# Healthcare-Robotics/assistive-gym

Measured on AMD Instinct MI355X. Metric: env_steps_per_sec, higher is better.
Workload: dtype f32; 1 GPU; FeedingJaco-v1, 4096 lockstep envs per MI355X, random-policy rollout, 5 simulation steps per env step, 50 PGS sweeps; envs_per_gpu=4096, global_envs=4096, reset_pool=256, reset=pool, parallelism=env-sharded x1, obs_allgather=False

## Files before the change

### __graft_entry__.py

```python
import os
import subprocess
import sys

ROOT = os.path.dirname(os.path.abspath(__file__))
if ROOT not in sys.path:
    sys.path.insert(0, ROOT)


def build():
    from assistive_gym_amd.build import build as build_lib
    build_lib(force=True)
    build_lib(out=os.path.join(ROOT, 'assistive_gym_amd', 'lib', 'variants', 'lvs.so'), extra=('-DAGX_PGS_LV=3',), only=['FEEDING'])
    build_lib(out=os.path.join(ROOT, 'assistive_gym_amd', 'lib', 'variants', 'scan4.so'), extra=('-DAGX_GJK_SCAN_WIDE=0', '-DAGX_GJK_SCAN_ONE=0'), only=['FEEDING'])
    subprocess.check_call(['make', '-C', os.path.join(ROOT, 'oracle')], stdout=subprocess.DEVNULL)
    if os.path.isdir('/root/reference/assistive_gym/envs/assets'):
        from assistive_gym_amd.model import compiler
        compiler.main()
    import assistive_gym_amd
    from assistive_gym_amd import libagx
    L = libagx.load()
    missing = [e for e in libagx.EXPORTS if not hasattr(L, e)]
    assert not missing, missing


def smoke():
    import numpy as np
    sys.path.insert(0, os.path.join(ROOT, 'tests'))
    from assistive_gym_amd import libagx
    from assistive_gym_amd.blob import ModelBlob
    from assistive_gym_amd.vec_env import build_reset_pool
    from oracle_lib import Oracle
    libagx.check(libagx.load().agx_selftest(0), 'agx_selftest')
    n = 64
    for model in ('feeding_jaco', 'bed_bathing_sawyer'):
        blob = ModelBlob.load(model)
        states = build_reset_pool(blob, n, seed=1001)
        st = libagx.Stepper(blob, n)
        st.set_state(states)
        actions = np.random.RandomState(0).uniform(-1, 1, (n, blob.act_dim)).astype(np.float32)
        obs, rew, done, info = st.step_host(actions)
        o = Oracle(blob)
        worst = 0.0
        for i in range(8):
            o_obs, o_rew, _, o_info = o.step(states[i].copy(), actions[i])
            worst = max(worst, float(np.abs(obs[i] - o_obs).max()), abs(float(rew[i]) - o_rew))
        assert np.isfinite(obs).all() and np.isfinite(rew).all()
# ... 10 lines not shown
```

### assistive_gym_amd/csrc/agx_collide.h

```cpp
#pragma once

namespace agx {

struct Cand { v3 pa, pb, n; float dist, gap; };
constexpr float GJK_FAR_MARGIN = 1e-4f;

AGX_DEV void make_shape(const Ctx& c, int col, v3 shift, gjk_shape& s) {
  s.n = CLI(c, col, AGX_C_NVERT);
  s.v = c.bf + c.o_vert + 3 * CLI(c, col, AGX_C_VOFF);
  v3 p; body_xf(c, CLI(c, col, AGX_C_BODY), s.R, p);
  s.p = p - shift; s.box = false;
  s.c = mul(s.R, mk3(CLF(c, col, AGX_C_AABB_C), CLF(c, col, AGX_C_AABB_C + 1), CLF(c, col, AGX_C_AABB_C + 2))) + s.p;
}
AGX_DEV bool narrowphase(const Ctx& c, int ca, int cb, float limit, Cand& out, bool has) {
  const float* AB = c.lds + L_ARENA;
  gjk_shape sa, sb;
  sa.v = nullptr; sa.n = 0; sa.box = false; sa.c = mk3(0.f, 0.f, 0.f); sb.v = nullptr; sb.n = 0; sb.box = false; sb.c = sa.c;
  v3 shift = mk3(0.f, 0.f, 0.f);
  float ra = 0.f, rb = 0.f;
  bool ok = has;
  if (has) {
    shift = mk3(0.5f * (AB[ABS * ca] + AB[ABS * ca + 3]), 0.5f * (AB[ABS * ca + 1] + AB[ABS * ca + 4]), 0.5f * (AB[ABS * ca + 2] + AB[ABS * ca + 5]));
    make_shape(c, ca, shift, sa); make_shape(c, cb, shift, sb);
    if (CLI(c, cb, AGX_C_BODY) == AGX_BODY_WORLD && sb.n == 8 && (CLI(c, cb, AGX_C_TAG) == AGX_TAG_TABLE || CLI(c, cb, AGX_C_TAG) == AGX_TAG_PLANE)) {
// ... 259 lines not shown
  const int na_live = nlive[0], nb = nlive[1];
  wave_sync();
  const int npairs = na_live * nb * rep;
  for (int base = 0; base < npairs; base += 64) {
    const int p = base + lane; bool ok = p < npairs;
    const int pq = ok ? p / rep : 0, sub = ok ? p - pq * rep : 0;
    const int ai = pq / nb; const int a = LIST[ai], b = LIST[128 + pq - ai * nb];
    ok = ok && (!same || b > a) && (sub == 0 || (face_box(c, b) && CLI(c, a, AGX_C_NVERT) >= 2));
    if (ok && no_adjacent) {
      const int la = CLI(c, a, AGX_C_BODY), lb = CLI(c, b, AGX_C_BODY);
      if (la == lb) ok = false;
      else if (la >= 0 && la < AGX_BODY_ROBOT_BASE && lb >= 0 && lb < AGX_BODY_ROBOT_BASE && (RBI(c, la, AGX_R_PARENT) == lb || RBI(c, lb, AGX_R_PARENT) == la)) ok = false;
    }
    if (ok) for (int q = 0; q < 3; q++) if (AB[ABS * a + q] > AB[ABS * b + 3 + q] + mg || AB[ABS * b + q] > AB[ABS * a + 3 + q] + mg) ok = false;
    if (ok) { const float reach = mg + rel_travel(c, a, b) + 1e-5f; ok = !sphere_box_apart(c, a, b, reach) && (CLI(c, a, AGX_C_NVERT) == 1 || !sphere_box_apart(c, b, a, reach)); }
    const uint64_t m = wave_ballot(ok);
    const int slot = wn + wave_rank(m);
    if (ok && slot < WL_CAP) WL[slot] = a | (b << 9) | (g << 18) | (sub << 24);
    wn += popc64(m);
  }
  wave_sync();
  return wn;
}

AGX_DEV void collide(Ctx& c) {
  float* L = c.lds; float* AB = L + L_ARENA; const int lane = c.lane;
  const float brk = PRM(c, AGX_P_CONTACT_BREAK), slack = PRM(c, AGX_P_CONTACT_SLACK);
  CollideState cs; cs.ncon = 0; cs.near_mask = 0; cs.overflow = 0; cs.nqpt = 0;
  cs.maxc = (int)PRM(c, AGX_P_MAX_CONTACTS); if (cs.maxc > MAX_CON) cs.maxc = MAX_CON;
  long long ct0 = c.timing ? wave_clock() : 0, ct1;
#define AGX_CTICK(k) if (c.timing) { ct1 = wave_clock(); c.tm[k] += ct1 - ct0; ct0 = ct1; }
  if (lane < MAX_DOF + MAX_FREE) {
    v3 w = mk3(0, 0, 0), v = w;
    if (lane < MAX_DOF) { if (lane < c.ndof) for (int d = lane; d >= 0; d = RBI(c, d, AGX_R_PARENT)) { const float qd = L[L_VEL + d]; w = w + qd * ld3(L + L_S + 6 * d); v = v + qd * ld3(L + L_S + 6 * d + 3); } }
    else if (lane - MAX_DOF < c.nfree) {
      const int fb = lane - MAX_DOF, o = c.ndof + 6 * fb;
      w = ld3(L + L_VEL + o + 3);
      v = ld3(L + L_VEL + o) + cross(w, ld3(L + L_MISC + M_REF) - ld3(L + L_ST + c.s_free + 13 * fb));
    }
    L[L_WMAG + lane] = sqrtf(dot(w, w));
    st3(AB + A_TW + 6 * lane, w); st3(AB + A_TW + 6 * lane + 3, v);
  }
  wave_sync();
  for (int col = lane; col < c.ncoll; col += 64) {
    const int code = CLI(c, col, AGX_C_BODY);
    m3 R; v3 p; body_xf(c, code, R, p);
    v3 cl = mk3(CLF(c, col, AGX_C_AABB_C), CLF(c, col, AGX_C_AABB_C + 1), CLF(c, col, AGX_C_AABB_C + 2));
    v3 hl = mk3(CLF(c, col, AGX_C_AABB_H), CLF(c, col, AGX_C_AABB_H + 1), CLF(c, col, AGX_C_AABB_H + 2));
    v3 cw = mul(R, cl) + p; float r = CLF(c, col, AGX_C_RADIUS);
    v3 vc = point_velocity(c, code, cw);
    const float wmag = body_wmag(c, code);
    const float grow = (sqrtf(dot(vc, vc)) + wmag * (sqrtf(dot(hl, hl)) + r)) * c.dt;
    for (int k = 0; k < 3; k++) {
      float h = fabsf(R.a[3 * k]) * hl.x + fabsf(R.a[3 * k + 1]) * hl.y + fabsf(R.a[3 * k + 2]) * hl.z + r;
      AB[ABS * col + k] = comp(cw, k) - h - grow; AB[ABS * col + 3 + k] = comp(cw, k) + h + grow;
    }
    AB[ABS * col + 6] = grow;
  }
  wave_sync();
  AGX_CTICK(8)
  const int gender = c.ldsi[L_ST + c.s_env + AGX_E_GENDER];
  uint64_t live_groups = 0;
  GroupRegs G; G.a0 = 0; G.a1 = 0; G.b0 = 0; G.b1 = 0; G.flags = 0; G.keep = 0;
  for (int k = 0; k < 3; k++) { G.alo[k] = 0.f; G.ahi[k] = 0.f; G.blo[k] = 0.f; G.bhi[k] = 0.f; }
  {
    const int g = lane; bool live = false;
    if (g < c.ngroup) {
// ... 56 lines not shown
```

### assistive_gym_amd/csrc/agx_ctx.h

```cpp
#pragma once

namespace agx {

#ifndef AGX_MAX_DOF
#define AGX_MAX_DOF 16
#endif
#ifndef AGX_MAX_FREE
#define AGX_MAX_FREE 10
#endif
#ifndef AGX_MAX_BLOCK
#define AGX_MAX_BLOCK 10
#endif
#ifndef AGX_TASK
#define AGX_TASK 0
#endif
#define AGX_HAS_SAMPLER 1
constexpr int MAX_DOF = AGX_MAX_DOF;
constexpr int MAX_FREE = AGX_MAX_FREE;
constexpr int MAX_BLOCK = AGX_MAX_BLOCK;
constexpr int TASK = AGX_TASK;
constexpr int MAX_HUMAN = 20;
constexpr int MAX_CON = 64;
constexpr int MAX_ROWS = 160;
#ifndef AGX_ST_WORDS
// ... 95 lines not shown
  float* lds; int* ldsi;
  int lane;
  int ndof, nfree, nhuman, ncoll, ngroup, nfood, nv;
  int nrobot, nhdof, gender, frozen, s_tremor;
  float limit_scale;
  bool coop;
  int o_params, o_robot, o_free, o_coll, o_vert, o_group, o_task, o_dirs;
  int s_q, s_qd, s_qt, s_free, s_base, s_human, s_env;
  float dt;
  bool hooks;
  int ncon, nrows, first_normal, near_mask, overflow;
  float* gqpt; int nqpt;
  float* dbg;
  float* E; float* H;
  int nent;
  float* gcon;
  long long tm[16]; bool timing;
};

#define PRM(c, k) ((c).bf[(c).o_params + (k)])
#define RREC(c, d) ((d) < (c).nrobot ? (d) : (d) + (c).gender * (c).nhdof)
#define RBF(c, d, k) ((c).bf[(c).o_robot + RREC(c, d) * AGX_R_STRIDE + (k)])
#define RBI(c, d, k) ((c).bi[(c).o_robot + RREC(c, d) * AGX_R_STRIDE + (k)])
#define DLO(c, d) (RBF(c, d, AGX_R_LOWER) * ((RBI(c, d, AGX_R_KIND) & 3) == 1 ? (c).limit_scale : 1.f))
#define DHI(c, d) (RBF(c, d, AGX_R_UPPER) * ((RBI(c, d, AGX_R_KIND) & 3) == 1 ? (c).limit_scale : 1.f))
#define FROZEN(c, d) ((d) < 32 && (((c).frozen >> (d)) & 1))
#define FBF(c, b, k) ((c).bf[(c).o_free + (b) * AGX_F_STRIDE + (k)])
#define CLF(c, i, k) ((c).bf[(c).o_coll + (i) * AGX_C_STRIDE + (k)])
#define CLI(c, i, k) ((c).bi[(c).o_coll + (i) * AGX_C_STRIDE + (k)])
#define GRI(c, g, k) ((c).bi[(c).o_group + (g) * AGX_G_STRIDE + (k)])
#define TKF(c, k) ((c).bf[(c).o_task + (k)])
#define TKI(c, k) ((c).bi[(c).o_task + (k)])

AGX_DEV void ctx_init(Ctx& c, const uint32_t* blob, float* lds, int lane) {
  c.bf = (const float*)blob; c.bi = (const int*)blob; c.lds = lds; c.ldsi = (int*)lds; c.lane = lane;
  const int* h = c.bi;
  c.ndof = h[AGX_H_NDOF]; c.nfree = h[AGX_H_NFREE]; c.nhuman = h[AGX_H_NHUMAN]; c.ncoll = h[AGX_H_NCOLL];
  c.ngroup = h[AGX_H_NGROUP]; c.nfood = h[AGX_H_NFOOD]; c.nv = c.ndof + 6 * c.nfree;
  c.o_params = h[AGX_H_OFF_PARAMS]; c.o_robot = h[AGX_H_OFF_ROBOT]; c.o_free = h[AGX_H_OFF_FREE]; c.o_coll = h[AGX_H_OFF_COLL];
  c.o_vert = h[AGX_H_OFF_VERT]; c.o_group = h[AGX_H_OFF_GROUP]; c.o_task = h[AGX_H_OFF_TASK]; c.o_dirs = h[AGX_H_OFF_DIRS];
  c.s_q = h[AGX_H_S_Q]; c.s_qd = h[AGX_H_S_QD]; c.s_qt = h[AGX_H_S_QT]; c.s_free = h[AGX_H_S_FREE]; c.s_base = h[AGX_H_S_BASE];
  c.s_human = h[AGX_H_S_HUMAN]; c.s_env = h[AGX_H_S_ENV]; c.s_tremor = h[AGX_H_S_TREMOR];
  c.nrobot = h[AGX_H_NROBOT]; c.nhdof = h[AGX_H_NHDOF]; c.gender = 0; c.frozen = 0; c.limit_scale = 1.f; c.coop = false;
  c.dt = PRM(c, AGX_P_DT) / (float)(h[AGX_H_SIM_SUBSTEPS] > 1 ? h[AGX_H_SIM_SUBSTEPS] : 1); c.hooks = true;
  c.ncon = 0; c.nrows = 0; c.first_normal = 0; c.near_mask = 0; c.overflow = 0; c.nent = 0; c.dbg = nullptr; c.E = nullptr; c.H = nullptr; c.gcon = nullptr; c.gqpt = nullptr; c.nqpt = 0;
  c.timing = false; for (int k = 0; k < 16; k++) c.tm[k] = 0;
}

AGX_DEV float dot6p(const float* a, const float* b) { return a[0] * b[0] + a[1] * b[1] + a[2] * b[2] + a[3] * b[3] + a[4] * b[4] + a[5] * b[5]; }
AGX_DEV void body_xf(const Ctx& c, int code, m3& R, v3& p) {
  const float* L = c.lds;
  if (code == AGX_BODY_WORLD) { R.a[0] = 1; R.a[1] = 0; R.a[2] = 0; R.a[3] = 0; R.a[4] = 1; R.a[5] = 0; R.a[6] = 0; R.a[7] = 0; R.a[8] = 1; p = mk3(0, 0, 0); }
  else if (code >= AGX_BODY_HUMAN0) { const float* h = L + L_HUMAN + 12 * (code - AGX_BODY_HUMAN0); p = ld3(h); R = ldm3(h + 3); }
  else if (code >= AGX_BODY_FREE0) { int b = code - AGX_BODY_FREE0; p = ld3(L + L_ST + c.s_free + 13 * b); R = ldm3(L + L_FREER + 9 * b); }
  else if (code == AGX_BODY_ROBOT_BASE) { p = ld3(L + L_BASE); R = ldm3(L + L_BASE + 3); }
  else { p = ld3(L + L_LINKP + 3 * code); R = ldm3(L + L_LINKR + 9 * code); }
}

}
```

### assistive_gym_amd/csrc/agx_dyn.h

```cpp
#pragma once

namespace agx {

AGX_DEV void kinematics(Ctx& c) {
  float* L = c.lds; const int lane = c.lane, n = c.ndof;
  for (int d = 0; d < n; d++) {
    int par = RBI(c, d, AGX_R_PARENT);
    v3 pp; m3 PR;
    if (par == AGX_PARENT_HUMAN_BASE) { pp = ld3(L + L_HUMAN); PR = ldm3(L + L_HUMAN + 3); }
    else if (par < 0) { pp = ld3(L + L_BASE); PR = ldm3(L + L_BASE + 3); } else { pp = ld3(L + L_LINKP + 3 * par); PR = ldm3(L + L_LINKR + 9 * par); }
    v3 tp = mk3(RBF(c, d, AGX_R_TPOS), RBF(c, d, AGX_R_TPOS + 1), RBF(c, d, AGX_R_TPOS + 2));
    m3 Rt = quat_to_m3(RBF(c, d, AGX_R_TQUAT), RBF(c, d, AGX_R_TQUAT + 1), RBF(c, d, AGX_R_TQUAT + 2), RBF(c, d, AGX_R_TQUAT + 3));
    v3 ax = mk3(RBF(c, d, AGX_R_AXIS), RBF(c, d, AGX_R_AXIS + 1), RBF(c, d, AGX_R_AXIS + 2));
    const bool prismatic = RBI(c, d, AGX_R_JTYPE) == 1;
    const float qj = L[L_ST + c.s_q + d];
    m3 R = mul(PR, Rt);
    v3 p = mul(PR, tp) + pp;
    if (prismatic) p = p + qj * mul(R, ax); else R = mul(R, axis_angle_m3(ax, qj));
    wave_sync();
    if (lane == 0) { st3(L + L_LINKP + 3 * d, p); stm3(L + L_LINKR + 9 * d, R); }
    wave_sync();
  }
  {
    int ee = TKI(c, AGX_T_EE_LINK);
    v3 lp = ld3(L + L_LINKP + 3 * ee); m3 LR = ldm3(L + L_LINKR + 9 * ee);
    v3 ep = mul(LR, mk3(TKF(c, AGX_T_EE_POS), TKF(c, AGX_T_EE_POS + 1), TKF(c, AGX_T_EE_POS + 2))) + lp;
    m3 ER = mul(LR, quat_to_m3(TKF(c, AGX_T_EE_QUAT), TKF(c, AGX_T_EE_QUAT + 1), TKF(c, AGX_T_EE_QUAT + 2), TKF(c, AGX_T_EE_QUAT + 3)));
    if (lane == 0) { st3(L + L_MISC + M_REF, lp); st3(L + L_MISC + M_EEP, ep); stm3(L + L_MISC + M_EER, ER); }
  }
  wave_sync();
  const v3 ref = ld3(L + L_MISC + M_REF);
  float* A = L + L_ARENA;
  if (lane < n) {
    const int d = lane;
    v3 p = ld3(L + L_LINKP + 3 * d) - ref; m3 R = ldm3(L + L_LINKR + 9 * d);
    v3 aw = mul(R, mk3(RBF(c, d, AGX_R_AXIS), RBF(c, d, AGX_R_AXIS + 1), RBF(c, d, AGX_R_AXIS + 2)));
    if (RBI(c, d, AGX_R_JTYPE) == 1) { st3(L + L_S + 6 * d, mk3(0.f, 0.f, 0.f)); st3(L + L_S + 6 * d + 3, aw); }
    else { st3(L + L_S + 6 * d, aw); st3(L + L_S + 6 * d + 3, cross(p, aw)); }
    v3 cw = mul(R, mk3(RBF(c, d, AGX_R_COM), RBF(c, d, AGX_R_COM + 1), RBF(c, d, AGX_R_COM + 2))) + p;
    st3(A + A_COMW + 3 * d, cw);
    m3 Il;
    Il.a[0] = RBF(c, d, AGX_R_INERTIA); Il.a[4] = RBF(c, d, AGX_R_INERTIA + 1); Il.a[8] = RBF(c, d, AGX_R_INERTIA + 2);
    Il.a[1] = Il.a[3] = RBF(c, d, AGX_R_INERTIA + 3); Il.a[2] = Il.a[6] = RBF(c, d, AGX_R_INERTIA + 4); Il.a[5] = Il.a[7] = RBF(c, d, AGX_R_INERTIA + 5);
    stm3(A + A_IW + 9 * d, mul_bt(mul(R, Il), R));
  }
  wave_sync();
  if (lane < n) {
    const int d = lane;
    float v[6] = {0, 0, 0, 0, 0, 0};
    for (int k = d; k >= 0; k = RBI(c, k, AGX_R_PARENT)) { float qd = L[L_ST + c.s_qd + k]; for (int j = 0; j < 6; j++) v[j] += L[L_S + 6 * k + j] * qd; }
    float qd = L[L_ST + c.s_qd + d];
    v3 w = mk3(v[0], v[1], v[2]), vo = mk3(v[3], v[4], v[5]);
    v3 sw = qd * ld3(L + L_S + 6 * d), sv = qd * ld3(L + L_S + 6 * d + 3);
    v3 ca = cross(w, sw), cl = cross(w, sv) + cross(vo, sw);
    for (int j = 0; j < 6; j++) A[A_VSP + 6 * d + j] = v[j];
    st3(A + A_CVP + 6 * d, ca); st3(A + A_CVP + 6 * d + 3, cl);
  }
  if (lane < c.nfree) {
    const int b = lane; const float* r = L + L_ST + c.s_free + 13 * b;
    m3 R = quat_to_m3(r[3], r[4], r[5], r[6]);
    stm3(L + L_FREER + 9 * b, R);
    m3 Di; for (int k = 0; k < 9; k++) Di.a[k] = 0;
    for (int k = 0; k < 3; k++) { float I = FBF(c, b, AGX_F_INERTIA + k); Di.a[4 * k] = I > 0 ? 1.0f / I : 0.0f; }
    stm3(L + L_FIINV + 9 * b, mul_bt(mul(R, Di), R));
  }
  wave_sync();
}

AGX_DEV float skewc(v3 c, int i, int j) {
  if (i == j) return 0.f;
  int k = 3 - i - j; float s = ((j - i + 3) % 3 == 1) ? -1.f : 1.f;
  return s * comp(c, k);
}
AGX_DEV void aba_and_minv(Ctx& c) {
  float* L = c.lds; float* A = L + L_ARENA; const int lane = c.lane, n = c.ndof;
  const float kl = PRM(c, AGX_P_LIN_DAMP), ka = PRM(c, AGX_P_ANG_DAMP);
  if (lane < 36) {
    const int r = lane / 6, cc = lane % 6;
    for (int d = 0; d < n; d++) {
      float m = RBF(c, d, AGX_R_MASS); v3 cw = ld3(A + A_COMW + 3 * d);
      float val;
      if (r < 3 && cc < 3) val = A[A_IW + 9 * d + 3 * r + cc] + m * ((r == cc ? dot(cw, cw) : 0.f) - comp(cw, r) * comp(cw, cc));
      else if (r < 3) val = m * skewc(cw, r, cc - 3);
      else if (cc < 3) val = m * skewc(cw, cc, r - 3);
      else val = (r == cc) ? m : 0.f;
      A[A_IA + 36 * d + lane] = val;
    }
  }
  if (lane < n) {
    const int d = lane;
    float m = RBF(c, d, AGX_R_MASS); v3 cw = ld3(A + A_COMW + 3 * d); m3 Iw = ldm3(A + A_IW + 9 * d);
    v3 w = ld3(A + A_VSP + 6 * d), vo = ld3(A + A_VSP + 6 * d + 3);
    v3 vc = vo + cross(w, cw);
    v3 hl = m * vc, ha = mul(Iw, w) + cross(cw, hl);
    v3 pa_ang = cross(w, ha) + cross(vo, hl), pa_lin = cross(w, hl);
    float sl = kl + kl * sqrtf(dot(vc, vc)), sa = ka + ka * sqrtf(dot(w, w));
    const float gz = PRM(c, (RBI(c, d, AGX_R_KIND) & 1) ? AGX_P_HUMAN_GRAVITY_Z : AGX_P_ROBOT_GRAVITY_Z);
    v3 f = mk3(0, 0, m * gz) - (m * sl) * vc;
    v3 tau = -(sa * mul(Iw, w));
    v3 fa = tau + cross(cw, f);
    st3(A + A_PA + 6 * d, pa_ang - fa); st3(A + A_PA + 6 * d + 3, pa_lin - f);
  }
  wave_sync();
  for (int d = n - 1; d >= 0; d--) {
    if (lane < 6) { float s = 0; for (int k = 0; k < 6; k++) s += A[A_IA + 36 * d + 6 * lane + k] * L[L_S + 6 * d + k]; A[A_U + 6 * d + lane] = s; }
    wave_sync();
    float D = dot6p(L + L_S + 6 * d, A + A_U + 6 * d);
    float Dinv = (D > 1e-30f && !FROZEN(c, d)) ? 1.0f / D : 0.0f;
    float u = -RBF(c, d, AGX_R_JDAMP) * L[L_ST + c.s_qd + d] - dot6p(L + L_S + 6 * d, A + A_PA + 6 * d);
    if (lane == 0) { A[A_DINV + d] = Dinv; A[A_UU + d] = u; }
    int par = RBI(c, d, AGX_R_PARENT);
    if (par >= 0) {
      float addp = 0.f;
      if (lane < 6) {
        float s = 0;
        for (int j = 0; j < 6; j++) s += (A[A_IA + 36 * d + 6 * lane + j] - A[A_U + 6 * d + lane] * A[A_U + 6 * d + j] * Dinv) * A[A_CVP + 6 * d + j];
        addp = A[A_PA + 6 * d + lane] + s + A[A_U + 6 * d + lane] * (u * Dinv);
      }
      if (lane < 36) { const int r = lane / 6, cc = lane % 6; A[A_IA + 36 * par + lane] += A[A_IA + 36 * d + lane] - A[A_U + 6 * d + r] * A[A_U + 6 * d + cc] * Dinv; }
      if (lane < 6) A[A_PA + 6 * par + lane] += addp;
    }
    wave_sync();
  }
  for (int d = 0; d < n; d++) {
    int par = RBI(c, d, AGX_R_PARENT);
    float ap[6];
    for (int k = 0; k < 6; k++) ap[k] = (par < 0 ? 0.f : A[A_ACC + 6 * par + k]) + A[A_CVP + 6 * d + k];
    float qdd = (A[A_UU + d] - dot6p(A + A_U + 6 * d, ap)) * A[A_DINV + d];
    wave_sync();
    if (lane == 0) { A[A_QDD + d] = qdd; for (int k = 0; k < 6; k++) A[A_ACC + 6 * d + k] = ap[k] + L[L_S + 6 * d + k] * qdd; }
    wave_sync();
  }
  if (lane < COLS_LANES) for (int j = lane; j < n; j += COLS_LANES) {
    const int b0 = j < c.nrobot ? 0 : c.nrobot, b1 = j < c.nrobot ? c.nrobot : n;
    float* P = A + A_COLS + lane * (MAX_BLOCK * 6);
    for (int k = 0; k < (b1 - b0) * 6; k++) P[k] = 0.f;
    float* UU = A + A_COLS + COLS_LANES * MAX_BLOCK * 6 + lane * MAX_BLOCK;
    for (int d = b1 - 1; d >= b0; d--) {
      float u = (d == j ? 1.f : 0.f) - dot6p(L + L_S + 6 * d, P + 6 * (d - b0));
      UU[d - b0] = u;
      int par = RBI(c, d, AGX_R_PARENT);
      if (par >= 0) { float s = u * A[A_DINV + d]; for (int k = 0; k < 6; k++) P[6 * (par - b0) + k] += P[6 * (d - b0) + k] + A[A_U + 6 * d + k] * s; }
    }
    for (int d = b0; d < b1; d++) {
      int par = RBI(c, d, AGX_R_PARENT);
      float ap[6]; for (int k = 0; k < 6; k++) ap[k] = par < 0 ? 0.f : P[6 * (par - b0) + k];
      float qdd = (UU[d - b0] - dot6p(A + A_U + 6 * d, ap)) * A[A_DINV + d];
      for (int k = 0; k < 6; k++) P[6 * (d - b0) + k] = ap[k] + L[L_S + 6 * d + k] * qdd;
      L[L_MINV + d * MAX_DOF + j] = qdd;
    }
    for (int d = 0; d < n; d++) if (d < b0 || d >= b1) L[L_MINV + d * MAX_DOF + j] = 0.f;
  }
  wave_sync();
  if (c.dbg && lane < n) { c.dbg[DBG_QDD + lane] = A[A_QDD + lane]; }
}

AGX_DEV void predict_velocities(Ctx& c) {
  float* L = c.lds; float* A = L + L_ARENA; const int lane = c.lane, n = c.ndof; const float dt = c.dt;
  for (int k = lane; k < 128; k += 64) L[L_VEL + k] = 0.f;
  wave_sync();
  if (lane < n) L[L_VEL + lane] = L[L_ST + c.s_qd + lane] + dt * A[A_QDD + lane];
  if (lane < c.nfree) {
    const int b = lane, o = n + 6 * b; const float* r = L + L_ST + c.s_free + 13 * b;
    v3 v = ld3(r + 7), w = ld3(r + 10);
    float kl = PRM(c, AGX_P_LIN_DAMP), ka = PRM(c, AGX_P_ANG_DAMP);
    float sl = kl + kl * sqrtf(dot(v, v)), sa = ka + ka * sqrtf(dot(w, w));
    v3 g = mk3(0, 0, FBF(c, b, AGX_F_GRAVITY));
    st3(L + L_VEL + o, v + dt * (g - sl * v));
    m3 R = ldm3(L + L_FREER + 9 * b), Ii = ldm3(L + L_FIINV + 9 * b);
    v3 wl = tmul(R, w);
    v3 Iw = mul(R, mk3(FBF(c, b, AGX_F_INERTIA) * wl.x, FBF(c, b, AGX_F_INERTIA + 1) * wl.y, FBF(c, b, AGX_F_INERTIA + 2) * wl.z));
    v3 acc = mul(Ii, -cross(w, Iw));
    st3(L + L_VEL + o + 3, w + dt * (acc - sa * w));
  }
  wave_sync();
}

AGX_DEV v3 point_velocity(const Ctx& c, int code, v3 x) {
  const float* L = c.lds;
  if (code >= 0 && code < AGX_BODY_ROBOT_BASE) {
    float sv[6] = {0, 0, 0, 0, 0, 0};
    for (int d = code; d >= 0; d = RBI(c, d, AGX_R_PARENT)) { float q = L[L_VEL + d]; for (int k = 0; k < 6; k++) sv[k] += L[L_S + 6 * d + k] * q; }
    v3 xr = x - ld3(L + L_MISC + M_REF);
    return mk3(sv[3], sv[4], sv[5]) + cross(mk3(sv[0], sv[1], sv[2]), xr);
  } else if (code >= AGX_BODY_FREE0 && code < AGX_BODY_HUMAN0) {
    int b = code - AGX_BODY_FREE0, o = c.ndof + 6 * b;
    v3 r = x - ld3(L + L_ST + c.s_free + 13 * b);
    return ld3(L + L_VEL + o) + cross(ld3(L + L_VEL + o + 3), r);
  }
  return mk3(0, 0, 0);
}

}
```

### assistive_gym_amd/csrc/agx_env.h

```cpp
#pragma once

namespace agx {

AGX_DEV void integrate(Ctx& c, const float* gvel, float dv0, float dv1) {
  float* L = c.lds; const int lane = c.lane, n = c.ndof; const float dt = c.dt;
  L[L_VEL + lane] = gvel[lane] + dv0;
  L[L_VEL + lane + 64] = gvel[lane + 64] + dv1;
  wave_sync();
  if (lane < n) {
    const int d = lane;
    float qd = L[L_VEL + d], q = L[L_ST + c.s_q + d] + dt * qd;
    if (c.hooks && (RBI(c, d, AGX_R_KIND) & 5) == 1 && !FROZEN(c, d)) {
      const float lo = DLO(c, d), hi = DHI(c, d);
      if (q < lo - AGX_LIMIT_EPS) { q = lo; qd = 0.f; } else if (q > hi + AGX_LIMIT_EPS) { q = hi; qd = 0.f; }
    }
    L[L_ST + c.s_qd + d] = qd; L[L_ST + c.s_q + d] = q;
  }
  if (lane < c.nfree) {
    const int b = lane, o = n + 6 * b; float* r = L + L_ST + c.s_free + 13 * b;
    v3 v = ld3(L + L_VEL + o), w = ld3(L + L_VEL + o + 3);
    st3(r + 7, v); st3(r + 10, w); st3(r, ld3(r) + dt * v);
    float wn = sqrtf(dot(w, w)), th = wn * dt; float dq[4];
    if (th > 1e-12f) { float sc = sinf(0.5f * th) / wn; dq[0] = w.x * sc; dq[1] = w.y * sc; dq[2] = w.z * sc; dq[3] = cosf(0.5f * th); }
    else { dq[0] = 0.5f * dt * w.x; dq[1] = 0.5f * dt * w.y; dq[2] = 0.5f * dt * w.z; dq[3] = 1.f; }
// ... 480 lines not shown
  float dv0 = 0.f, dv1 = 0.f;
  bool solved = false;
  if constexpr (LVW_COMPILED) { if (lvw_eligible(c, lds_words)) solved = pgs_lvw(c, lds, lds_words, dv0, dv1); }
  if constexpr (LVS_COMPILED) { if (!solved && lvs_eligible(c, lds_words)) { pgs_lvs(c, lds, lds_words, dv0, dv1); solved = true; } }
  if (!solved) {
    const bool rowspace = RS_MAX_ROWS > 0 && c.nrows <= RS_MAX_ROWS && c.nv <= 64 && c.nv <= RS_NVP && c.nrows > 0 && c.nent <= SOLVE_LDS_PAIRS;
    { const int np = c.nent < SOLVE_LDS_PAIRS ? c.nent : SOLVE_LDS_PAIRS;
      const f2* src = (const f2*)scr.ent; f2* dst = (f2*)(lds + L_SOLVE_ENT);
      for (int k = lane; k < np; k += 64) dst[k] = src[k]; }
    wave_sync();
    if (!(rowspace && pgs_rowspace(c, lds + L_SOLVE_ENT, dv0, dv1))) pgs(c, dv0, dv1);
  }
  warm_remember(c, scr, lane);
  const long long t1 = gdebug ? wave_clock() : 0;
  solve_tail(c, gstate, scr, sw, phase, dv0, dv1);
  if (gdebug && lane == 0) { gdebug[DBG_TIME + 5] = (float)(t1 - t0); gdebug[DBG_TIME + 6] = (float)(wave_clock() - t1); }
}

AGX_DEV void observe_dressing(const Ctx& c, float cloth_force_sum, float robot_force, float* gobs);
AGX_DEV void env_observe(const uint32_t* blob, float* gstate, float* gobs, float* lds, int lane) {
  Ctx c; ctx_init(c, blob, lds, lane);
  load_env(c, gstate, c.bi[AGX_H_STATE_WORDS]);
  kinematics(c); update_target(c);
  if constexpr (TASK == AGX_TASK_BED_BATHING) observe_bed(c, 0.f, 0.f, 0.f, gobs);
  else if constexpr (TASK == AGX_TASK_SCRATCH_ITCH) observe_scratch(c, 0.f, 0.f, 0.f, gobs);
  else if constexpr (TASK == AGX_TASK_DRESSING) observe_dressing(c, c.lds[L_ST + c.bi[AGX_H_S_TASK] + AGX_DR_FORCE_SUM], 0.f, gobs);
  else if constexpr (TASK == AGX_TASK_ARM_MANIPULATION) observe_arm(c, 0.f, 0.f, 0.f, 0.f, 0.f, gobs);
  else observe(c, 0.f, 0.f, gobs);
}

AGX_DEV float frame_speed(const Ctx& c, int link, v3 p) {
  const float* L = c.lds;
  float sv[6] = {0, 0, 0, 0, 0, 0};
  for (int d = link; d >= 0; d = RBI(c, d, AGX_R_PARENT)) { float qd = L[L_ST + c.s_qd + d]; for (int j = 0; j < 6; j++) sv[j] += L[L_S + 6 * d + j] * qd; }
  v3 xr = p - ld3(L + L_MISC + M_REF);
  v3 v = mk3(sv[3], sv[4], sv[5]) + cross(mk3(sv[0], sv[1], sv[2]), xr);
  return sqrtf(dot(v, v));
}
AGX_DEV float ee_speed_of(const Ctx& c) { return frame_speed(c, TKI(c, AGX_T_EE_LINK), ld3(c.lds + L_MISC + M_EEP)); }

AGX_DEV void env_finish_bed(const uint32_t* blob, float* gstate, const float* gaction, float* gscratch, float* gobs, float* greward, uint8_t* gdone,
                            float* ginfo, float* lds, int lane) {
  Ctx c; ctx_init(c, blob, lds, lane);
  float* L = c.lds; int* Li = c.ldsi;
  const int sw = c.bi[AGX_H_STATE_WORDS], act_dim = c.bi[AGX_H_ACT_DIM];
  Scratch scr = scratch_of(gscratch);
  c.ncon = scr.meta[META_NCON]; c.nrows = scr.meta[META_NROWS]; c.first_normal = scr.meta[META_NNC]; c.nqpt = scr.meta[META_NQPT];
  load_env(c, gstate, sw);
  float an2 = 0.f;
  for (int k = 0; k < act_dim; k++) an2 += gaction[k] * gaction[k];
  wave_sync();
  kinematics(c);
  float rf = 0.f, tf = 0.f, thf = 0.f, pf = 0.f;
  if (lane < c.ncon) {
    const float* k = scr.con + CON_STRIDE * lane; const int* ki = (const int*)k;
    const int ca = ki[C_CA], cb = ki[C_CB], ta = CLI(c, ca, AGX_C_TAG), tb = CLI(c, cb, AGX_C_TAG);
    const float f = k[C_LAM] / c.dt;
    const bool human = ta == AGX_TAG_HUMAN || tb == AGX_TAG_HUMAN, tool = ta == AGX_TAG_TOOL || tb == AGX_TAG_TOOL, robot = ta == AGX_TAG_ROBOT || tb == AGX_TAG_ROBOT;
    if (tool) tf = f;
    if (human && robot) rf = f;
    if (human && tool) { thf = f; const int tc = ta == AGX_TAG_TOOL ? ca : cb; if (TKI(c, AGX_T_PAD_LINK) >> (CLI(c, tc, AGX_C_LINK) + 1) & 1) pf = f; }
  }
  const float robot_f = wave_sum(rf), tool_f = wave_sum(tf), pad_f = wave_sum(pf), total_f = robot_f + wave_sum(thf);
  observe_bed(c, tool_f, total_f, pad_f, gobs);
  int success = Li[L_ST + c.s_env + AGX_E_TASK_SUCCESS];
  const int s_task = c.bi[AGX_H_S_TASK];
  int new_points = 0;
// ... 577 lines not shown
```

### assistive_gym_amd/csrc/agx_gjk.h

```cpp
#pragma once

struct gjk_shape {
  const float* v;
  int n;
  m3 R;
  v3 p;
  v3 c;
  bool box;
  v3 lo, hi;
};

AGX_DEV float gjk_dot3(float x, float y, float z, v3 d) { return fmaf(z, d.z, fmaf(y, d.y, x * d.x)); }
AGX_DEV v3 gjk_local_dir(const m3& R, v3 d) {
  return mk3(fmaf(R.a[6], d.z, fmaf(R.a[3], d.y, R.a[0] * d.x)), fmaf(R.a[7], d.z, fmaf(R.a[4], d.y, R.a[1] * d.x)), fmaf(R.a[8], d.z, fmaf(R.a[5], d.y, R.a[2] * d.x)));
}
AGX_DEV v3 gjk_vertex0(const gjk_shape& s) {
  if (s.box) return s.lo;
  return mul(s.R, mk3(s.v[0], s.v[1], s.v[2])) + s.p;
}
#ifndef AGX_GJK_SCAN_WIDE
#define AGX_GJK_SCAN_WIDE 2
#endif
#if AGX_GJK_SCAN_WIDE != 0 && AGX_GJK_SCAN_WIDE != 2
#error "AGX_GJK_SCAN_WIDE: 0 or 2"
#endif
#ifndef AGX_GJK_SCAN_ONE
#define AGX_GJK_SCAN_ONE 1
#endif

AGX_DEV v3 gjk_support(const gjk_shape& s, v3 d) {
  if (s.box) {
    v3 best = s.lo; float bd = dot(s.lo, d);
    for (int q = 1; q < 8; q++) {
      v3 c = mk3((q & 4) ? s.hi.x : s.lo.x, (q & 2) ? s.hi.y : s.lo.y, (q & 1) ? s.hi.z : s.lo.z);
      float t = dot(c, d);
      if (t > bd) { bd = t; best = c; }
    }
    return best;
  }
  const v3 dl = gjk_local_dir(s.R, d);
  const float* V = s.v;
#if AGX_GJK_SCAN_WIDE
  const int last = s.n - 1;
  float bd = -3.0e38f; int best = 0;
#define GJK_LDV(j, kk) const int i##j = (kk) < last ? (kk) : last; const float x##j = V[3 * i##j], y##j = V[3 * i##j + 1], z##j = V[3 * i##j + 2];
#define GJK_CMP(j) { const float t = gjk_dot3(x##j, y##j, z##j, dl); if (t > bd) { bd = t; best = i##j; } }
  int k = 0;
#if AGX_GJK_SCAN_ONE
  if (s.n > 1)
#endif
  {
  for (; s.n - k > 4; k += 8) {
    GJK_LDV(0, k) GJK_LDV(1, k + 1) GJK_LDV(2, k + 2) GJK_LDV(3, k + 3) GJK_LDV(4, k + 4) GJK_LDV(5, k + 5) GJK_LDV(6, k + 6) GJK_LDV(7, k + 7)
    GJK_CMP(0) GJK_CMP(1) GJK_CMP(2) GJK_CMP(3) GJK_CMP(4) GJK_CMP(5) GJK_CMP(6) GJK_CMP(7)
  }
  if (k < s.n) {
    GJK_LDV(0, k) GJK_LDV(1, k + 1) GJK_LDV(2, k + 2) GJK_LDV(3, k + 3)
    GJK_CMP(0) GJK_CMP(1) GJK_CMP(2) GJK_CMP(3)
  }
  }
// ... 121 lines not shown
    if (!any) return true;
  }
  const bool k0 = l[0] > 0, k1 = l[1] > 0, k2 = l[2] > 0, k3 = l[3] > 0;
  const int c0 = k0 ? 1 : 0, c1 = c0 + (k1 ? 1 : 0), c2 = c1 + (k2 ? 1 : 0), cnt = c2 + (k3 ? 1 : 0);
  const int i0 = k0 ? 0 : (k1 ? 1 : (k2 ? 2 : 3));
  const int i1 = (k1 && c1 == 2) ? 1 : ((k2 && c2 == 2) ? 2 : 3);
  const int i2 = (k2 && c2 == 3) ? 2 : 3;
  const gjk_pt q0 = gjk_sel(i0, s.p0, s.p1, s.p2, s.p3), q1 = gjk_sel(i1, s.p0, s.p1, s.p2, s.p3), q2 = gjk_sel(i2, s.p0, s.p1, s.p2, s.p3);
  const float m0 = gjk_self(i0, l[0], l[1], l[2], l[3]), m1 = gjk_self(i1, l[0], l[1], l[2], l[3]), m2 = gjk_self(i2, l[0], l[1], l[2], l[3]);
  s.p0 = q0; s.p1 = q1; s.p2 = q2;
  s.l0 = m0; s.l1 = cnt > 1 ? m1 : 0.f; s.l2 = cnt > 2 ? m2 : 0.f; s.l3 = 0.f;
  s.n = cnt;
  v = s.l0 * s.p0.w;
  if (cnt > 1) v = v + s.l1 * s.p1.w;
  if (cnt > 2) v = v + s.l2 * s.p2.w;
  return false;
}

AGX_DEV bool gjk_distance(const gjk_shape& sa, const gjk_shape& sb, float tol, int maxit, float far, bool has, float& dist, v3& pa, v3& pb) {
  gjk_simplex s;
  v3 d0 = sa.c - sb.c;
  float dd = dot(d0, d0);
  if (!(dd >= 1e-12f)) { d0 = mk3(1.f, 0.f, 0.f); dd = 1.f; }
  const v3 a0 = gjk_support_wave(sa, -d0, has), b0 = gjk_support_wave(sb, d0, has);
  v3 v = a0 - b0;
  float vv = dot(v, v);
  s.p0.a = a0; s.p0.b = b0; s.p0.w = v; s.p1 = s.p0; s.p2 = s.p0; s.p3 = s.p0;
  s.n = 1; s.l0 = 1; s.l1 = 0; s.l2 = 0; s.l3 = 0;
  pa = a0; pb = b0;
  bool pen = false, far_out = false, active = has;
  float lb = 0.f;
  int my_iters = 0; (void)my_iters;
  { const float vw0 = dot(d0, v); if (has && vw0 > 0.f && vw0 * vw0 > far * far * dd) { far_out = true; lb = vw0 / sqrtf(dd); active = false; } }
  for (int it = 0; it < maxit; it++) {
    if (active && vv < 1e-12f) { pen = true; active = false; }
    if (!wave_any(active)) break;
    const v3 wa = gjk_support_wave(sa, -v, active), wb = gjk_support_wave(sb, v, active);
    if (active) {
      my_iters++;
      const v3 w = wa - wb;
      const float vw = dot(v, w);
      const bool e0 = s.p0.w.x == w.x && s.p0.w.y == w.y && s.p0.w.z == w.z;
      const bool e1 = s.n > 1 && s.p1.w.x == w.x && s.p1.w.y == w.y && s.p1.w.z == w.z;
      const bool e2 = s.n > 2 && s.p2.w.x == w.x && s.p2.w.y == w.y && s.p2.w.z == w.z;
      if (vw > 0.f && vw * vw > far * far * vv) { far_out = true; lb = vw / sqrtf(vv); active = false; }
      else if (vv - vw <= tol * vv || e0 || e1 || e2) active = false;
      else {
        gjk_pt np; np.w = w; np.a = wa; np.b = wb;
        if (s.n == 1) s.p1 = np; else if (s.n == 2) s.p2 = np; else s.p3 = np;
        s.n++;
        v3 vn;
        if (gjk_solve(s, vn)) { pen = !(vw > 0.f); active = false; }
        else {
          const float vvn = dot(vn, vn);
          if (vvn >= vv) active = false;
          else {
            v = vn; vv = vvn;
            pa = s.l0 * s.p0.a; pb = s.l0 * s.p0.b;
            if (s.n > 1) { pa = pa + s.l1 * s.p1.a; pb = pb + s.l1 * s.p1.b; }
            if (s.n > 2) { pa = pa + s.l2 * s.p2.a; pb = pb + s.l2 * s.p2.b; }
          }
        }
      }
    }
  }
  AGX_TRACE_GJK(has, my_iters, sa.n, sb.n, sb.box, far_out, far_out ? lb : sqrtf(vv), far)
  if (pen) { dist = 0; return true; }
  dist = far_out ? lb : sqrtf(vv);
  return false;
}

AGX_DEV void gjk_penetration(const gjk_shape& sa, const gjk_shape& sb, const float* dirs, int ndir, float& depth, v3& n, v3& pa, v3& pb) {
  float best = 3.0e38f; int bi = 0;
  for (int k = 0; k < ndir; k++) {
    v3 d = mk3(dirs[3 * k], dirs[3 * k + 1], dirs[3 * k + 2]);
    v3 a = gjk_support(sa, -d), b = gjk_support(sb, d);
    float dep = dot(b, d) - dot(a, d);
    if (dep < best) { best = dep; bi = k; }
  }
  n = mk3(dirs[3 * bi], dirs[3 * bi + 1], dirs[3 * bi + 2]);
  pa = gjk_support(sa, -n);
  pb = pa + best * n;
  depth = best;
}
```

Measured before the change: 611,500 env-steps/s.

## Add lean build: ancestor bitmasks, register-cached link params, single-point GJK shortcut

Kinematic chain walks now iterate a precomputed ancestor bitmask held in LDS instead of chasing parent indices through the global model blob. Per-link joint parameters are loaded once per lane into registers and broadcast across the wave inside the serial kinematics and ABA loops. GJK distance and penetration skip recomputing support points for single-vertex shapes. The new path is on by default behind AGX_BUILD_LEAN, with a non-lean variant library built for comparison. The cost is extra register pressure and a reliance on the ancestor mask layout fitting in 64 bits.

```diff
diff --git a/__graft_entry__.py b/__graft_entry__.py
--- a/__graft_entry__.py
+++ b/__graft_entry__.py
@@ -12,6 +12,7 @@
     build_lib(force=True)
     build_lib(out=os.path.join(ROOT, 'assistive_gym_amd', 'lib', 'variants', 'lvs.so'), extra=('-DAGX_PGS_LV=3',), only=['FEEDING'])
     build_lib(out=os.path.join(ROOT, 'assistive_gym_amd', 'lib', 'variants', 'scan4.so'), extra=('-DAGX_GJK_SCAN_WIDE=0', '-DAGX_GJK_SCAN_ONE=0'), only=['FEEDING'])
+    build_lib(out=os.path.join(ROOT, 'assistive_gym_amd', 'lib', 'variants', 'lean0.so'), extra=('-DAGX_BUILD_LEAN=0',))
     subprocess.check_call(['make', '-C', os.path.join(ROOT, 'oracle')], stdout=subprocess.DEVNULL)
     if os.path.isdir('/root/reference/assistive_gym/envs/assets'):
         from assistive_gym_amd.model import compiler
diff --git a/assistive_gym_amd/csrc/agx_collide.h b/assistive_gym_amd/csrc/agx_collide.h
--- a/assistive_gym_amd/csrc/agx_collide.h
+++ b/assistive_gym_amd/csrc/agx_collide.h
@@ -315,7 +315,11 @@
 #define AGX_CTICK(k) if (c.timing) { ct1 = wave_clock(); c.tm[k] += ct1 - ct0; ct0 = ct1; }
   if (lane < MAX_DOF + MAX_FREE) {
     v3 w = mk3(0, 0, 0), v = w;
+#if AGX_BUILD_LEAN
+    if (lane < MAX_DOF) { if (lane < c.ndof) for (uint64_t m = chain_of(c, lane); m; ) { const int d = chain_pop(m); const float qd = L[L_VEL + d]; w = w + qd * ld3(L + L_S + 6 * d); v = v + qd * ld3(L + L_S + 6 * d + 3); } }
+#else
     if (lane < MAX_DOF) { if (lane < c.ndof) for (int d = lane; d >= 0; d = RBI(c, d, AGX_R_PARENT)) { const float qd = L[L_VEL + d]; w = w + qd * ld3(L + L_S + 6 * d); v = v + qd * ld3(L + L_S + 6 * d + 3); } }
+#endif
     else if (lane - MAX_DOF < c.nfree) {
       const int fb = lane - MAX_DOF, o = c.ndof + 6 * fb;
       w = ld3(L + L_VEL + o + 3);
diff --git a/assistive_gym_amd/csrc/agx_ctx.h b/assistive_gym_amd/csrc/agx_ctx.h
--- a/assistive_gym_amd/csrc/agx_ctx.h
+++ b/assistive_gym_amd/csrc/agx_ctx.h
@@ -151,6 +151,20 @@
 #define TKF(c, k) ((c).bf[(c).o_task + (k)])
 #define TKI(c, k) ((c).bi[(c).o_task + (k)])
 
+#ifndef AGX_BUILD_LEAN
+#define AGX_BUILD_LEAN 1
+#endif
+#if AGX_BUILD_LEAN != 0 && AGX_BUILD_LEAN != 1
+#error "AGX_BUILD_LEAN: 0 or 1"
+#endif
+AGX_DEV uint64_t chain_of(const Ctx& c, int d) {
+  uint64_t m = (uint32_t)c.ldsi[L_MISC + M_ANC + ANC_WORDS * d];
+  if (ANC_WORDS == 2) m |= (uint64_t)(uint32_t)c.ldsi[L_MISC + M_ANC + 2 * d + 1] << 32;
+  return m;
+}
+AGX_DEV int chain_pop(uint64_t& m) { const int k = 63 - clz64(m); m &= ~(1ull << k); return k; }
+AGX_DEV int chain_parent(const Ctx& c, int d) { const uint64_t m = chain_of(c, d) & ~(1ull << d); return m ? 63 - clz64(m) : -1; }
+
 AGX_DEV void ctx_init(Ctx& c, const uint32_t* blob, float* lds, int lane) {
   c.bf = (const float*)blob; c.bi = (const int*)blob; c.lds = lds; c.ldsi = (int*)lds; c.lane = lane;
   const int* h = c.bi;
diff --git a/assistive_gym_amd/csrc/agx_dyn.h b/assistive_gym_amd/csrc/agx_dyn.h
--- a/assistive_gym_amd/csrc/agx_dyn.h
+++ b/assistive_gym_amd/csrc/agx_dyn.h
@@ -1,18 +1,39 @@
 #pragma once
 
 namespace agx {
+
+struct LinkRegs { int parent, jtype; float tpos[3], tquat[4], axis[3], mass, jdamp; };
 
 AGX_DEV void kinematics(Ctx& c) {
   float* L = c.lds; const int lane = c.lane, n = c.ndof;
+#if AGX_BUILD_LEAN
+  LinkRegs K; K.parent = -1; K.jtype = 0; K.mass = 0.f; K.jdamp = 0.f; for (int k = 0; k < 3; k++) { K.tpos[k] = 0.f; K.axis[k] = 0.f; } for (int k = 0; k < 4; k++) K.tquat[k] = 0.f;
+  if (lane < n) {
+    K.parent = RBI(c, lane, AGX_R_PARENT); K.jtype = RBI(c, lane, AGX_R_JTYPE);
+    for (int k = 0; k < 3; k++) { K.tpos[k] = RBF(c, lane, AGX_R_TPOS + k); K.axis[k] = RBF(c, lane, AGX_R_AXIS + k); }
+    for (int k = 0; k < 4; k++) K.tquat[k] = RBF(c, lane, AGX_R_TQUAT + k);
+  }
+#endif
   for (int d = 0; d < n; d++) {
+#if AGX_BUILD_LEAN
+    const int par = wave_bcast_i(K.parent, d);
+#else
     int par = RBI(c, d, AGX_R_PARENT);
+#endif
     v3 pp; m3 PR;
     if (par == AGX_PARENT_HUMAN_BASE) { pp = ld3(L + L_HUMAN); PR = ldm3(L + L_HUMAN + 3); }
     else if (par < 0) { pp = ld3(L + L_BASE); PR = ldm3(L + L_BASE + 3); } else { pp = ld3(L + L_LINKP + 3 * par); PR = ldm3(L + L_LINKR + 9 * par); }
+#if AGX_BUILD_LEAN
+    v3 tp = mk3(wave_bcast(K.tpos[0], d), wave_bcast(K.tpos[1], d), wave_bcast(K.tpos[2], d));
+    m3 Rt = quat_to_m3(wave_bcast(K.tquat[0], d), wave_bcast(K.tquat[1], d), wave_bcast(K.tquat[2], d), wave_bcast(K.tquat[3], d));
+    v3 ax = mk3(wave_bcast(K.axis[0], d), wave_bcast(K.axis[1], d), wave_bcast(K.axis[2], d));
+    const bool prismatic = wave_bcast_i(K.jtype, d) == 1;
+#else
     v3 tp = mk3(RBF(c, d, AGX_R_TPOS), RBF(c, d, AGX_R_TPOS + 1), RBF(c, d, AGX_R_TPOS + 2));
     m3 Rt = quat_to_m3(RBF(c, d, AGX_R_TQUAT), RBF(c, d, AGX_R_TQUAT + 1), RBF(c, d, AGX_R_TQUAT + 2), RBF(c, d, AGX_R_TQUAT + 3));
     v3 ax = mk3(RBF(c, d, AGX_R_AXIS), RBF(c, d, AGX_R_AXIS + 1), RBF(c, d, AGX_R_AXIS + 2));
     const bool prismatic = RBI(c, d, AGX_R_JTYPE) == 1;
+#endif
     const float qj = L[L_ST + c.s_q + d];
     m3 R = mul(PR, Rt);
     v3 p = mul(PR, tp) + pp;
@@ -48,7 +69,11 @@
   if (lane < n) {
     const int d = lane;
     float v[6] = {0, 0, 0, 0, 0, 0};
+#if AGX_BUILD_LEAN
+    for (uint64_t m = chain_of(c, d); m; ) { const int k = chain_pop(m); float qd = L[L_ST + c.s_qd + k]; for (int j = 0; j < 6; j++) v[j] += L[L_S + 6 * k + j] * qd; }
+#else
     for (int k = d; k >= 0; k = RBI(c, k, AGX_R_PARENT)) { float qd = L[L_ST + c.s_qd + k]; for (int j = 0; j < 6; j++) v[j] += L[L_S + 6 * k + j] * qd; }
+#endif
     float qd = L[L_ST + c.s_qd + d];
     v3 w = mk3(v[0], v[1], v[2]), vo = mk3(v[3], v[4], v[5]);
     v3 sw = qd * ld3(L + L_S + 6 * d), sv = qd * ld3(L + L_S + 6 * d + 3);
@@ -75,10 +100,20 @@
 AGX_DEV void aba_and_minv(Ctx& c) {
   float* L = c.lds; float* A = L + L_ARENA; const int lane = c.lane, n = c.ndof;
   const float kl = PRM(c, AGX_P_LIN_DAMP), ka = PRM(c, AGX_P_ANG_DAMP);
+#if AGX_BUILD_LEAN
+  LinkRegs K; K.parent = -1; K.mass = 0.f; K.jdamp = 0.f;
+  if (lane < n) { K.parent = RBI(c, lane, AGX_R_PARENT); K.mass = RBF(c, lane, AGX_R_MASS); K.jdamp = RBF(c, lane, AGX_R_JDAMP); }
+  for (int d = 0; d < n; d++) {
+    const float m = wave_bcast(K.mass, d);
+    if (lane < 36) {
+      const int r = lane / 6, cc = lane % 6;
+      v3 cw = ld3(A + A_COMW + 3 * d);
+#else
   if (lane < 36) {
     const int r = lane / 6, cc = lane % 6;
     for (int d = 0; d < n; d++) {
       float m = RBF(c, d, AGX_R_MASS); v3 cw = ld3(A + A_COMW + 3 * d);
+#endif
       float val;
       if (r < 3 && cc < 3) val = A[A_IW + 9 * d + 3 * r + cc] + m * ((r == cc ? dot(cw, cw) : 0.f) - comp(cw, r) * comp(cw, cc));
       else if (r < 3) val = m * skewc(cw, r, cc - 3);
@@ -89,7 +124,12 @@
   }
   if (lane < n) {
     const int d = lane;
-    float m = RBF(c, d, AGX_R_MASS); v3 cw = ld3(A + A_COMW + 3 * d); m3 Iw = ldm3(A + A_IW + 9 * d);
+#if AGX_BUILD_LEAN
+    float m = K.mass;
+#else
+    float m = RBF(c, d, AGX_R_MASS);
+#endif
+    v3 cw = ld3(A + A_COMW + 3 * d); m3 Iw = ldm3(A + A_IW + 9 * d);
     v3 w = ld3(A + A_VSP + 6 * d), vo = ld3(A + A_VSP + 6 * d + 3);
     v3 vc = vo + cross(w, cw);
     v3 hl = m * vc, ha = mul(Iw, w) + cross(cw, hl);
@@ -107,9 +147,15 @@
     wave_sync();
     float D = dot6p(L + L_S + 6 * d, A + A_U + 6 * d);
     float Dinv = (D > 1e-30f && !FROZEN(c, d)) ? 1.0f / D : 0.0f;
+#if AGX_BUILD_LEAN
+    float u = -wave_bcast(K.jdamp, d) * L[L_ST + c.s_qd + d] - dot6p(L + L_S + 6 * d, A + A_PA + 6 * d);
+    if (lane == 0) { A[A_DINV + d] = Dinv; A[A_UU + d] = u; }
+    const int par = wave_bcast_i(K.parent, d);
+#else
     float u = -RBF(c, d, AGX_R_JDAMP) * L[L_ST + c.s_qd + d] - dot6p(L + L_S + 6 * d, A + A_PA + 6 * d);
     if (lane == 0) { A[A_DINV + d] = Dinv; A[A_UU + d] = u; }
     int par = RBI(c, d, AGX_R_PARENT);
+#endif
     if (par >= 0) {
       float addp = 0.f;
       if (lane < 6) {
@@ -123,7 +169,11 @@
     wave_sync();
   }
   for (int d = 0; d < n; d++) {
+#if AGX_BUILD_LEAN
+    const int par = wave_bcast_i(K.parent, d);
+#else
     int par = RBI(c, d, AGX_R_PARENT);
+#endif
     float ap[6];
     for (int k = 0; k < 6; k++) ap[k] = (par < 0 ? 0.f : A[A_ACC + 6 * par + k]) + A[A_CVP + 6 * d + k];
     float qdd = (A[A_UU + d] - dot6p(A + A_U + 6 * d, ap)) * A[A_DINV + d];
@@ -139,11 +189,19 @@
     for (int d = b1 - 1; d >= b0; d--) {
       float u = (d == j ? 1.f : 0.f) - dot6p(L + L_S + 6 * d, P + 6 * (d - b0));
       UU[d - b0] = u;
+#if AGX_BUILD_LEAN
+      const int par = chain_parent(c, d);
+#else
       int par = RBI(c, d, AGX_R_PARENT);
+#endif
       if (par >= 0) { float s = u * A[A_DINV + d]; for (int k = 0; k < 6; k++) P[6 * (par - b0) + k] += P[6 * (d - b0) + k] + A[A_U + 6 * d + k] * s; }
     }
     for (int d = b0; d < b1; d++) {
+#if AGX_BUILD_LEAN
+      const int par = chain_parent(c, d);
+#else
       int par = RBI(c, d, AGX_R_PARENT);
+#endif
       float ap[6]; for (int k = 0; k < 6; k++) ap[k] = par < 0 ? 0.f : P[6 * (par - b0) + k];
       float qdd = (UU[d - b0] - dot6p(A + A_U + 6 * d, ap)) * A[A_DINV + d];
       for (int k = 0; k < 6; k++) P[6 * (d - b0) + k] = ap[k] + L[L_S + 6 * d + k] * qdd;
@@ -180,7 +238,11 @@
   const float* L = c.lds;
   if (code >= 0 && code < AGX_BODY_ROBOT_BASE) {
     float sv[6] = {0, 0, 0, 0, 0, 0};
+#if AGX_BUILD_LEAN
+    for (uint64_t m = chain_of(c, code); m; ) { const int d = chain_pop(m); float q = L[L_VEL + d]; for (int k = 0; k < 6; k++) sv[k] += L[L_S + 6 * d + k] * q; }
+#else
     for (int d = code; d >= 0; d = RBI(c, d, AGX_R_PARENT)) { float q = L[L_VEL + d]; for (int k = 0; k < 6; k++) sv[k] += L[L_S + 6 * d + k] * q; }
+#endif
     v3 xr = x - ld3(L + L_MISC + M_REF);
     return mk3(sv[3], sv[4], sv[5]) + cross(mk3(sv[0], sv[1], sv[2]), xr);
   } else if (code >= AGX_BODY_FREE0 && code < AGX_BODY_HUMAN0) {
diff --git a/assistive_gym_amd/csrc/agx_env.h b/assistive_gym_amd/csrc/agx_env.h
--- a/assistive_gym_amd/csrc/agx_env.h
+++ b/assistive_gym_amd/csrc/agx_env.h
@@ -536,7 +536,11 @@
 AGX_DEV float frame_speed(const Ctx& c, int link, v3 p) {
   const float* L = c.lds;
   float sv[6] = {0, 0, 0, 0, 0, 0};
+#if AGX_BUILD_LEAN
+  for (uint64_t m = chain_of(c, link); m; ) { const int d = chain_pop(m); float qd = L[L_ST + c.s_qd + d]; for (int j = 0; j < 6; j++) sv[j] += L[L_S + 6 * d + j] * qd; }
+#else
   for (int d = link; d >= 0; d = RBI(c, d, AGX_R_PARENT)) { float qd = L[L_ST + c.s_qd + d]; for (int j = 0; j < 6; j++) sv[j] += L[L_S + 6 * d + j] * qd; }
+#endif
   v3 xr = p - ld3(L + L_MISC + M_REF);
   v3 v = mk3(sv[3], sv[4], sv[5]) + cross(mk3(sv[0], sv[1], sv[2]), xr);
   return sqrtf(dot(v, v));
diff --git a/assistive_gym_amd/csrc/agx_gjk.h b/assistive_gym_amd/csrc/agx_gjk.h
--- a/assistive_gym_amd/csrc/agx_gjk.h
+++ b/assistive_gym_amd/csrc/agx_gjk.h
@@ -26,6 +26,9 @@
 #endif
 #ifndef AGX_GJK_SCAN_ONE
 #define AGX_GJK_SCAN_ONE 1
+#endif
+#ifndef AGX_BUILD_LEAN
+#define AGX_BUILD_LEAN 1
 #endif
 
 AGX_DEV v3 gjk_support(const gjk_shape& s, v3 d) {
@@ -213,10 +216,21 @@
   float lb = 0.f;
   int my_iters = 0; (void)my_iters;
   { const float vw0 = dot(d0, v); if (has && vw0 > 0.f && vw0 * vw0 > far * far * dd) { far_out = true; lb = vw0 / sqrtf(dd); active = false; } }
+#if AGX_BUILD_LEAN
+  const bool a_one = sa.n == 1 && !sa.box;
+#endif
   for (int it = 0; it < maxit; it++) {
     if (active && vv < 1e-12f) { pen = true; active = false; }
     if (!wave_any(active)) break;
+#if AGX_BUILD_LEAN
+    const bool a_need = active && !(a_one && it > 0);
+    v3 wa = s.p3.a;
+    if (wave_any(a_need)) { const v3 t = gjk_support_wave(sa, -v, a_need); if (a_need) wa = t; }
+    if (it == 0) s.p3.a = wa;
+    const v3 wb = gjk_support_wave(sb, v, active);
+#else
     const v3 wa = gjk_support_wave(sa, -v, active), wb = gjk_support_wave(sb, v, active);
+#endif
     if (active) {
       my_iters++;
       const v3 w = wa - wb;
@@ -253,9 +267,19 @@
 
 AGX_DEV void gjk_penetration(const gjk_shape& sa, const gjk_shape& sb, const float* dirs, int ndir, float& depth, v3& n, v3& pa, v3& pb) {
   float best = 3.0e38f; int bi = 0;
+#if AGX_BUILD_LEAN
+  const bool a_one = sa.n == 1 && !sa.box;
+  v3 a_pt = mk3(0.f, 0.f, 0.f);
+#endif
   for (int k = 0; k < ndir; k++) {
     v3 d = mk3(dirs[3 * k], dirs[3 * k + 1], dirs[3 * k + 2]);
+#if AGX_BUILD_LEAN
+    v3 a = a_pt;
+    if (!a_one || k == 0) { a = gjk_support(sa, -d); a_pt = a; }
+    v3 b = gjk_support(sb, d);
+#else
     v3 a = gjk_support(sa, -d), b = gjk_support(sb, d);
+#endif
     float dep = dot(b, d) - dot(a, d);
     if (dep < best) { best = dep; bi = k; }
   }
```

Result: no change. 617,100 env-steps/s (median of 6 runs) (+0.9%).
